# anhtu293/nndepth

Measured on AMD Instinct MI355X. Metric: stereo pairs/sec at 544x960, 32 iters (RAFT-Stereo), higher is better.
Workload: dtype f32 carried as 2 range-scaled fp16 pieces per operand (3 MFMA products, fp32 accumulate); 1 GPU; RAFT-Stereo base (ctx 64), 544x960, 32 iters, batch 1 per GPU, all 32 up_disp emitted; parallelism=single, launch=direct

## Files before the change

### nndepth_amd/csrc/common.h

```cpp
#pragma once
#include <hip/hip_runtime.h>
#include <atomic>
#include <cstdarg>
#include <cstdio>
#include "../../include/nndepth_amd.h"
#include "split_arith.h"

namespace nnd {

void set_error(const char* fmt, ...);

#define NND_HIP_CHECK(expr)                                                              \
    do {                                                                                 \
        hipError_t _e = (expr);                                                          \
        if (_e != hipSuccess) {                                                          \
            nnd::set_error("%s failed: %s (%s:%d)", #expr, hipGetErrorString(_e), __FILE__, __LINE__); \
            return NND_ERR_HIP;                                                          \
        }                                                                                \
    } while (0)

#define NND_LAUNCH_CHECK()                                                               \
    do {                                                                                 \
        hipError_t _e = hipGetLastError();                                               \
        if (_e != hipSuccess) {                                                          \
// ... 97 lines not shown
struct ConvLayer {
    int KH, KW, Cin, Cout, CI_T;
    int stride = 1;
    int arith = 0;
    bool range_scaled() const { return split_range_scaled(arith); }
    int64_t s_off = -1;
    int nchunks;
    int ncb;
    int64_t w_off, b_off;
    int64_t w_floats() const {
        return arith ? (int64_t)ncb * nchunks * KH * KW * arith * 256
                     : (int64_t)ncb * nchunks * KH * KW * CI_T * 32;
    }
    int64_t b_floats() const { return (int64_t)ncb * 32 + (range_scaled() ? 4 : 0); }
    double flops(int B, int H, int W) const { return 2.0 * B * H * W * (double)Cout * Cin * KH * KW; }
    int64_t tail_off() const { return b_off + (int64_t)ncb * 32; }
};

struct Act {
    float* ptr;
    int64_t bstride;
    int C;
};

struct ConvIO {
    Act src0, src1;
    Act out0, out1;
    Act aux0, aux1;
    Act bmap;
    int hidden = 0;
    float scale = 1.f;
    int Hin = 0, Win = 0;
    int flags = 0;
    bool src_tiled = false;
    bool dst_tiled = false;
    bool src_c4 = false;
    bool dst_c4 = false;
    int cout_need = 0;
    int force_ks = 0;
};

static inline bool conv_shape_built(int KH, int KW) { return (KH == 1 && (KW == 1 || KW == 5)) || (KW == 1 && KH == 5) || (KH == 3 && KW == 3); }

int conv_ci_t(int KH, int KW, int Cin, int stride = 1, int Cout = 0);

int launch_conv(const ConvLayer& L, const float* blob, const ConvIO& io, int epi,
                int B, int H, int W, hipStream_t stream);

void pack_conv(const ConvLayer& L, int nparts, const float* const* w, const float* const* b,
               const int* cout, float* blob, const int* ci_map = nullptr, int cin_src = 0);

bool conv_split_supported(int KH, int KW, int Cin, int stride, int arith, int Cout = 0);
int launch_conv_split(const ConvLayer& L, const float* blob, const ConvIO& io, int epi, int B, int H, int W, hipStream_t stream);
bool flow_branch_supported(const ConvLayer& f2, int fc);
int launch_flow_branch(const ConvLayer& f2, const float* blob, const float* w7t, const float* b7, const float* flow, int64_t fbs,
                       int fc, const ConvIO& io, int B, int H, int W, hipStream_t stream);
void pack_conv_split(const ConvLayer& L, int nparts, const float* const* w, const float* const* b, const int* cout, float* blob,
                     const int* ci_map, int cin_src);

bool enc_block_supported(const ConvLayer& c1, const ConvLayer& c2, const ConvLayer& ds);
int enc_block_launch(const ConvLayer& c1, const float* blob1, const ConvLayer& c2, const float* blob2, const ConvLayer& ds, const float* blobd,
                     const float* x, float* out, int N, int H, int W, hipStream_t stream);

bool thin3d_supported(int Cout, int stride);
bool slab3d_supported(int Cout, int C0, int C1, int stride, int arith);
int64_t slab3d_packed_floats(int Cout, int Ct, int stride);
void slab3d_pack(int Cout, int Ct, int stride, const float* w, const float* scale, const float* shift, float* out);
int slab3d_forward(int Cout, int C0, int C1, int stride, const float* packed, const float* x0, const float* x1, float* y, int N, int D,
                   int H, int W, float slope, hipStream_t s);
int64_t thin3d_packed_floats(int Cout, int Ct);
void thin3d_pack(int Cout, int Ct, const float* w, const float* scale, const float* shift, float* out);
int thin3d_forward(int Cout, int C0, int C1, int stride, const float* packed, const float* x0, const float* x1, float* y, int N, int D,
                   int H, int W, float slope, hipStream_t s);

int corr1d_lookup_launch(const float* pyr, const float* coords, float* out, int B, int H, int W, int num_levels,
                         int radius, hipStream_t stream, bool tiled);
int group_lookup_flat_launch(const float* pyr, const float* coords, float* out, int B, int G, int H, int W, int num_levels, int radius,
                             hipStream_t stream, bool tiled);
int igev_lookup_launch(const float* feat_pyramid, const float* geo_pyramid, const float* coords, float* out, int B, int G, int H,
                       int W, int num_levels, int radius, hipStream_t stream, bool tiled);
int convex_upsample_launch(const float* flow, const float* mask, float* out, int B, int C, int H, int W, int rate,
                           hipStream_t stream, bool tiled);

int agcl_iter_launch(const float* f1, const float* f2, const float* flow, float* warped, float* out, int N, int C, int H,
                     int W, int small_patch, hipStream_t s, bool tiled);
int agcl_offset_launch(const float* f1, const float* f2, const float* flow, const float* extra, float* out, int N, int C, int H,
                       int W, int small_patch, hipStream_t s, bool tiled);
int agcl_check(const char* what, int N, int C, int H, int W);
bool agcl_offset_cl_supported(int C);
int agcl_offset_cl_launch(const float* f1c, const float* f2c, const float* flow, const float* extra, float* out, int N, int C,
                          int H, int W, int small_patch, hipStream_t s, bool tiled);
int nchw_to_nhwc_launch(const float* in, float* out, int N, int C, int P, hipStream_t s);
int lookup_convc1_launch(const float* pyr, const float* geo, int G, const float* coords, const ConvLayer& L, const float* blob,
                         float* c1, int64_t c1_bs, int B, int H, int W, int num_levels, int radius, hipStream_t stream, bool c1_c4);
bool flow_branch_lookup_supported(int arith);
int flow_branch_lookup_launch(const ConvLayer& f2, const float* blob, const float* w7t, const float* b7, const float* flow, int64_t fbs,
                              int fc, const ConvIO& io, const float* pyr, const float* coords, const ConvLayer& Lc1, float* c1,
                              int64_t c1_bs, int B, int H, int W, int num_levels, int radius, hipStream_t stream, bool c1_c4);
bool igev_lookup_convc1_il_supported(int G, int num_levels, int radius);
int igev_lookup_convc1_il_launch(const float* il, int G, const float* coords, const ConvLayer& L, const float* blob, float* c1,
                                 int64_t c1_bs, int B, int H, int W, int num_levels, int radius, hipStream_t stream, bool c1_c4);
struct MaskUpFlowHead {
    const float* x;
    long xbs;
    int hid;
    const float* w;
    const float* bias;
    const float* coords_in;
    float *coords_out, *flow_out, *delta_out;
    float* hx_flow;
    long hx_bs;
    int hx_pm;
    int absolute;
};

// ... 8 lines not shown
```

### nndepth_amd/csrc/conv_split.hip

```cpp
#include "conv_launch.h"
#include "conv_split_kernel.h"
#include "flow_branch.h"

#include <atomic>
#include <cmath>
#include <cstdlib>
#include <cstring>

namespace nnd {

namespace {
uint16_t f16_rn(float x) {
    const _Float16 h = (_Float16)x;
    uint16_t u;
    memcpy(&u, &h, 2);
    return u;
}
float f16_to_f(uint16_t u) {
    _Float16 h;
    memcpy(&h, &u, 2);
    return (float)h;
}
uint16_t bf16_rn(float x) {
    uint32_t u;
// ... 57 lines not shown
                    size_t lds = (size_t)2 * ks * P * subb;
                    const size_t red = ks > 1 ? (size_t)waves * P * 4096 : 0;
                    if (red > lds) lds = red;
                    if (lds > 160 * 1024) continue;
                    const int max_waves = P > 2 ? 8 : SPLIT_MAX_WAVES;
                    int wg_per_cu = (int)((160 * 1024) / lds);
                    if (wg_per_cu > max_waves / waves) wg_per_cu = max_waves / waves;
                    if (wg_per_cu < 1) wg_per_cu = 1;
                    const double rounds = std::ceil((double)px_wgs * ny / (256.0 * wg_per_cu));
                    const double simd_waves = std::ceil(waves * wg_per_cu / 4.0);
                    double t = rounds * simd_waves * cdiv(L.nchunks, ks) * P / 2.0;
                    t *= 1.0 + 0.03 * (ks - 1);
                    t *= 1.0 + 0.02 * (4 - (wco < 4 ? wco : 4));
                    if (nu > 2 && P == 2) t *= 1.2;
                    if (t < best) {
                        best = t;
                        *out = {ny, wco, ks, P, ntiles, tiles_x, split_nu_variant(nu), fast, lds, STR};
                        found = true;
                    }
                }
            }
        }
        return found;
    };
    if (try_ks2 && search(force_ny, 2, force_p)) return true;
    if (search(force_ny, force_ks, force_p)) return true;
    return rule && search(-1, -1, -1);
}

bool restrict_split(const ConvLayer& L, int cout_need, SplitCfg* cfg) {
    const int npos = split_patch(L.KH, L.KW, L.arith, L.stride).NPOS;
    auto units = [&](int wco) { return split_staging_units(cfg->P, npos, cfg->ks, wco * cfg->ks); };
    if (!conv_restrict_cout(L, cout_need, &cfg->ny, &cfg->wco, [&](int wco) { return cfg->P == 2 && units(wco) <= 4; })) return false;
    cfg->nu = split_nu_variant(units(cfg->wco));
    return true;
}

bool split_fast_ok(const ConvLayer& L) { return !switches().split_no_fast || L.stride == 2; }
bool plan_split(const ConvLayer& L, const ConvIO& io, int B, int H, int W, SplitCfg* cfg) {
    if (!pick_split(L, io.src0.C, io.src1.C, B, H, W, split_fast_ok(L), cfg)) return false;
    cfg->restricted = restrict_split(L, io.cout_need, cfg);
    cfg->grid = dim3(cdiv(cfg->ntiles, cfg->P), cfg->ny, B), cfg->block = dim3(64 * cfg->wco * cfg->ks);
    return true;
}

void print_split_plan(const ConvLayer& L, const ConvIO& io, const SplitCfg& cfg) {
    fprintf(stderr, "[nnd] conv_split %dx%d Cin=%d Cout=%d pieces=%d: ny=%d, wco=%d, ks=%d, P=%d, nu=%d%s, grid %ux%ux%u, lds %zu B%s%s\n", L.KH,
            L.KW, L.Cin, L.Cout, L.arith, cfg.ny, cfg.wco, cfg.ks, cfg.P, cfg.nu, cfg.fast ? ", fast" : "", cfg.grid.x, cfg.grid.y, cfg.grid.z, cfg.lds,
            io.cout_need > 0 ? (cfg.restricted ? ", restricted to the wanted output channels" : ", whole layer (not restrictable)") : "",
            L.stride == 2 ? ", stride 2" : "");
}
}

extern template int launch_split_ns<1>(const ConvArgs&, const SplitCfg&, int, int, hipStream_t);
extern template int launch_split_ns<2>(const ConvArgs&, const SplitCfg&, int, int, hipStream_t);
extern template int launch_split_ns<3>(const ConvArgs&, const SplitCfg&, int, int, hipStream_t);

bool conv_split_supported(int KH, int KW, int Cin, int stride, int arith, int Cout) {
    if ((arith != 3 && arith != 2 && arith != 1) || (stride != 1 && stride != 2) || Cin % 16 != 0) return false;
    if (stride == 2) return ((KH == 3 && KW == 3) || (KH == 1 && KW == 1)) && Cout >= 96;
    return conv_shape_built(KH, KW);
}

int launch_conv_split(const ConvLayer& L, const float* blob, const ConvIO& io, int epi, int B, int H, int W, hipStream_t stream) {
    int rc, Hin, Win;
    NND_REQUIRE(conv_split_supported(L.KH, L.KW, L.Cin, L.stride, L.arith, L.Cout), "conv_split: %dx%d Cin=%d Cout=%d stride %d arith %d not built",
                L.KH, L.KW, L.Cin, L.Cout, L.stride, L.arith);
    NND_TRY(conv_check_io("conv_split", L, io, epi, H, W, &Hin, &Win));
    NND_REQUIRE(L.CI_T == 16 && L.nchunks * 16 == L.Cin, "conv_split: layer was not planned for 16-channel chunks");
    NND_REQUIRE(L.stride == 1 || io.src1.C == 0, "conv_split: stride 2 is built for one source");
    NND_REQUIRE((long)(L.Cin + 64) * tiled_plane(Hin, Win) < (1L << 31), "conv_split: plane offsets exceed 32 bits");
    SplitCfg cfg;
    NND_REQUIRE(plan_split(L, io, B, H, W, &cfg),
                "conv_split: no configuration for %dx%d Cin=%d (%d+%d) Cout=%d stride %d (NND_SPLIT_CFG ny=%d ks=%d P=%d%s)", L.KH, L.KW,
                L.Cin, io.src0.C, io.src1.C, L.Cout, L.stride, switches().split_ny, switches().split_ks, switches().split_p,
                split_fast_ok(L) ? "" : ", NND_SPLIT_NO_FAST");
    ConvArgs a;
    conv_fill_args(L, blob, io, epi, H, W, Hin, Win, &a);
    a.tiles_x = cfg.tiles_x; a.wco = cfg.wco; a.ks = cfg.ks; a.npos = cfg.ntiles;
#ifdef NND_DBG_STAMPS
    {
        static std::atomic<int> launches{0};
        static const int only = getenv("NND_DBG_STAMP_LAUNCH") ? atoi(getenv("NND_DBG_STAMP_LAUNCH")) : -1;
        const int idx = launches.fetch_add(1);
        a.dbg_stamp = only < 0 || idx == only;
    }
#endif
    if (calibrating() && split_range_scaled(L.arith))
        for (const Act* src : {&io.src0, &io.src1}) NND_TRY(calib_amax_act(*src, a.ls, B, Hin, Win, blob + L.tail_off(), stream));
    if (switches().conv_verbose) print_split_plan(L, io, cfg);
    rc = L.arith == 3   ? launch_split_ns<3>(a, cfg, L.KH, L.KW, stream)
         : L.arith == 2 ? launch_split_ns<2>(a, cfg, L.KH, L.KW, stream)
                        : launch_split_ns<1>(a, cfg, L.KH, L.KW, stream);
    NND_REQUIRE(rc != NND_ERR_UNSUPPORTED, "conv_split: shape %dx%d P=%d nu=%d %s is not instantiated", L.KH, L.KW, cfg.P, cfg.nu, cfg.fast ? "fast" : "generic");
    if (rc != NND_OK) return rc;
    NND_LAUNCH_CHECK();
    return NND_OK;
}

void pack_conv_split(const ConvLayer& L, int nparts, const float* const* w, const float* const* bvec, const int* cout, float* blob,
                     const int* ci_map, int cin_src) {
    if (!ci_map) cin_src = L.Cin;
    const int NT = L.KH * L.KW, NS = L.arith;
    uint16_t* wp = reinterpret_cast<uint16_t*>(blob + L.w_off);
    float* bp = blob + L.b_off;
    memset(wp, 0, sizeof(float) * L.w_floats());
// ... 97 lines not shown
```

### nndepth_amd/csrc/enc_block.hip

```cpp
#include "common.h"
#include "conv_epilogue.h"
#include "conv_split_kernel.h"
#include "layout.h"
#include "split_arith.h"

#include <atomic>

namespace nnd {

namespace {
constexpr int EB_TH = 8, EB_TW = 16;
constexpr int EB_YR = EB_TH + 2, EB_YC = EB_TW + 2;
constexpr int EB_XR = EB_TH + 4, EB_XC = EB_TW + 4;
constexpr int EB_NY = EB_YR * EB_YC, EB_NX = EB_XR * EB_XC;
constexpr int EB_NCH = 4;
constexpr int EB_B1 = 6, EB_B2 = 4;
constexpr int EB_HV = 2;
static_assert(EB_B1 * 32 >= EB_NY && EB_B2 * 32 == EB_TH * EB_TW, "column blocks cover the y region / the tile");
constexpr int eb_ps(int NS) { return NS * 32 + 16; }
constexpr size_t eb_lds_bytes(int NS) { return (size_t)(EB_NCH * EB_NY + EB_NX) * eb_ps(NS); }

struct EncBlockArgs {
    const float* x;
    float* out;
    long bs;
    const uint4 *w1, *w2;
    const float4* wd;
    const float *shift1, *scale1, *shift2, *scale2, *shiftd, *scaled;
    Lay lay;
    int H, W, tiles_x;
};

template <int NS, int P, int RW, int PAR>
__device__ __forceinline__ void eb_walk_chunk(const uint4* wc, const uint4* wn, uint4 (&ab)[2][3][NS], const unsigned char* const (&bb)[P],
                                              f32x16 (&acc)[P]) {
    constexpr int PS = eb_ps(NS), NUNIT = 9 * P;
    uint4 b[2][NS];
    auto read_b = [&](int u, uint4(&dst)[NS]) {
        const int t = u / P, pp = u % P;
#pragma unroll
        for (int s = 0; s < NS; ++s) dst[s] = *reinterpret_cast<const uint4*>(bb[pp] + ((t / 3) * RW + t % 3) * PS + s * 32);
    };
    read_b(0, b[0]);
#pragma unroll
    for (int dy = 0; dy < 3; ++dy) {
        uint4(&cur)[3][NS] = ab[(PAR + dy) & 1];
        uint4(&nxt)[3][NS] = ab[(PAR + dy + 1) & 1];
        const uint4* wr = dy < 2 ? wc + (dy + 1) * 3 * NS * 64 : wn;
#pragma unroll
        for (int dx = 0; dx < 3; ++dx)
#pragma unroll
            for (int s = 0; s < NS; ++s) nxt[dx][s] = wr[(dx * NS + s) * 64];
        __builtin_amdgcn_sched_barrier(0);
#pragma unroll
        for (int dx = 0; dx < 3; ++dx)
#pragma unroll
            for (int pp = 0; pp < P; ++pp) {
                const int u = (dy * 3 + dx) * P + pp;
                if (u + 1 < NUNIT) read_b(u + 1, b[(u + 1) & 1]);
                __builtin_amdgcn_sched_barrier(0);
                split_mfma_step<NS>(cur[dx], b[u & 1], acc[pp]);
                __builtin_amdgcn_sched_barrier(0);
            }
    }
}

template <int NS>
__global__ void __launch_bounds__(128 * EB_HV) __attribute__((amdgpu_waves_per_eu(EB_HV))) enc_block_kernel(EncBlockArgs a) {
    constexpr int EB_P1 = EB_B1 / EB_HV, EB_P2 = EB_B2 / EB_HV, NTHR = 128 * EB_HV, NU = (2 * EB_NX + NTHR - 1) / NTHR;
    constexpr int PS = eb_ps(NS), YCH = EB_NY * PS, CHW = 9 * NS * 64;
    extern __shared__ __attribute__((aligned(16))) unsigned char lds_raw[];
    unsigned char* const ybuf = lds_raw;
    unsigned char* const xbuf = lds_raw + EB_NCH * YCH;

    const int tid = threadIdx.x, lane = tid & 63;
    const int wave = __builtin_amdgcn_readfirstlane(tid >> 6);
    const int cb = wave & 1, half = wave >> 1;
    const int h2 = lane >> 5, l31 = lane & 31;
    const int b = blockIdx.z;
    const int ty0 = (blockIdx.x / a.tiles_x) * EB_TH, tx0 = (blockIdx.x % a.tiles_x) * EB_TW;
    const int H = a.H, W = a.W;
    const int SP = (int)a.lay.plane;
    const float* xs = a.x + b * a.bs;

    int goff[NU], gstep[NU], loff[NU];
    bool inimg[NU], own[NU];
#pragma unroll
    for (int i = 0; i < NU; ++i) {
        const int u = tid + i * NTHR;
        own[i] = u < 2 * EB_NX;
        const int oct = u / EB_NX, pos = u % EB_NX;
        const int gy = ty0 - 2 + pos / EB_XC, gx = tx0 - 2 + pos % EB_XC;
        inimg[i] = own[i] && gy >= 0 && gy < H && gx >= 0 && gx < W;
        goff[i] = inimg[i] ? oct * 8 * SP + (int)pix_off(a.lay, gy, gx) : 0;
        gstep[i] = inimg[i] ? 4 * SP : 0;
        loff[i] = pos * PS + oct * 16;
    }
    float stage[NU][8];
    auto stage_load = [&](int K) {
        const float* src = xs + (long)K * 16 * SP;
#pragma unroll
        for (int i = 0; i < NU; ++i)
#pragma unroll
            for (int g = 0; g < 2; ++g) {
                const float4 t = *reinterpret_cast<const float4*>(src + (unsigned)(goff[i] + g * gstep[i]));
                stage[i][4 * g] = t.x; stage[i][4 * g + 1] = t.y; stage[i][4 * g + 2] = t.z; stage[i][4 * g + 3] = t.w;
            }
    };
    const float* tail1 = a.shift1 + 64;
    const float* tail2 = a.shift2 + 64;
    const float oscale1 = tail1[SPLIT_TAIL_OSCALE], xscale1 = tail1[SPLIT_TAIL_XSCALE];
    const float oscale2 = tail2[SPLIT_TAIL_OSCALE], xscale2 = tail2[SPLIT_TAIL_XSCALE];
    auto stage_store = [&]() {
#pragma unroll
        for (int i = 0; i < NU; ++i) {
            float v[8];
#pragma unroll
            for (int j = 0; j < 8; ++j) v[j] = inimg[i] ? stage[i][j] : 0.f;
            uint4 pieces[NS];
            split_pieces<NS>(v, pieces, xscale1);
            if (own[i]) {
#pragma unroll
                for (int s = 0; s < NS; ++s) *reinterpret_cast<uint4*>(xbuf + loff[i] + s * 32) = pieces[s];
            }
        }
    };

    const unsigned char* xb1[EB_P1];
    int ypos[EB_P1];
    bool ywrite[EB_P1], yin[EB_P1];
#pragma unroll
    for (int pp = 0; pp < EB_P1; ++pp) {
        const int p = (half * EB_P1 + pp) * 32 + l31;
        const int pc = min(p, EB_NY - 1);
        const int yr = pc / EB_YC, yc = pc % EB_YC;
        ypos[pp] = pc;
        ywrite[pp] = p < EB_NY;
        const int iy = ty0 - 1 + yr, ix = tx0 - 1 + yc;
        yin[pp] = iy >= 0 && iy < H && ix >= 0 && ix < W;
        xb1[pp] = xbuf + (yr * EB_XC + yc) * PS + h2 * 16;
    }
    const uint4* w1 = a.w1 + (size_t)cb * EB_NCH * CHW + lane;
    const uint4* w2 = a.w2 + (size_t)cb * EB_NCH * CHW + lane;

    uint4 ab[2][3][NS];
#pragma unroll
    for (int dx = 0; dx < 3; ++dx)
#pragma unroll
        for (int s = 0; s < NS; ++s) ab[0][dx][s] = w1[(dx * NS + s) * 64];
    stage_load(0);
    stage_store();
    __syncthreads();

    f32x16 acc1[EB_P1];
#pragma unroll
    for (int pp = 0; pp < EB_P1; ++pp)
#pragma unroll
        for (int i = 0; i < 16; ++i) acc1[pp][i] = 0.f;

    auto conv1_chunk = [&](int K, auto par_c) {
        constexpr int PAR = decltype(par_c)::value;
        const bool more = K + 1 < EB_NCH;
        if (more) stage_load(K + 1);
        eb_walk_chunk<NS, EB_P1, EB_XC, PAR>(w1 + K * CHW, more ? w1 + (K + 1) * CHW : w2, ab, xb1, acc1);
        __syncthreads();
        if (more) {
            stage_store();
            __syncthreads();
        }
    };
    for (int K = 0; K < EB_NCH; K += 2) {
        conv1_chunk(K, std::integral_constant<int, 0>{});
        conv1_chunk(K + 1, std::integral_constant<int, 1>{});
    }

    {
        float sc1[16], sh1[16];
#pragma unroll
        for (int reg = 0; reg < 16; ++reg) {
            const int co = cb * 32 + (reg & 3) + 8 * (reg >> 2) + 4 * h2;
            sc1[reg] = a.scale1[co];
            sh1[reg] = a.shift1[co];
        }
#pragma unroll
        for (int pp = 0; pp < EB_P1; ++pp) {
#pragma unroll
            for (int q = 0; q < 4; ++q) {
                float v[4];
#pragma unroll
                for (int i = 0; i < 4; ++i) {
                    const float ac = acc1[pp][4 * q + i] * oscale1;
                    const float t = relu_nan(fmaf(ac, sc1[4 * q + i], sh1[4 * q + i]));
                    v[i] = yin[pp] ? t : 0.f;
                }
                uint2 pieces[NS];
                split_pieces_n<NS, 4, uint2>(v, pieces, xscale2);
                if (ywrite[pp]) {
                    unsigned char* d = ybuf + (cb * 2 + (q >> 1)) * YCH + ypos[pp] * PS + ((q & 1) * 8 + 4 * h2) * 2;
#pragma unroll
                    for (int s = 0; s < NS; ++s) *reinterpret_cast<uint2*>(d + s * 32) = pieces[s];
                }
            }
        }
    }
    __syncthreads();

    const int pxl = lane_pixel(l31), r2 = pxl >> 4, c2 = pxl & 15;
    int oy[EB_P2];
    const int ox = tx0 + c2;
    int yb2[EB_P2];
#pragma unroll
    for (int pp = 0; pp < EB_P2; ++pp) {
        const int row = 2 * (half * EB_P2 + pp) + r2;
        oy[pp] = ty0 + row;
        yb2[pp] = (row * EB_YC + c2) * PS + h2 * 16;
    }
    f32x16 acc2[EB_P2];
#pragma unroll
    for (int pp = 0; pp < EB_P2; ++pp)
#pragma unroll
        for (int i = 0; i < 16; ++i) acc2[pp][i] = 0.f;
    float4 xq[EB_P2][8], afr[8];
    auto conv2_chunk = [&](int K, auto par_c) {
        constexpr int PAR = decltype(par_c)::value;
        const unsigned char* bb[EB_P2];
#pragma unroll
        for (int pp = 0; pp < EB_P2; ++pp) bb[pp] = ybuf + K * YCH + yb2[pp];
        eb_walk_chunk<NS, EB_P2, EB_YC, PAR>(w2 + K * CHW, w2 + (K + 1 < EB_NCH ? K + 1 : K) * CHW, ab, bb, acc2);
    };
    conv2_chunk(0, std::integral_constant<int, 0>{});
    conv2_chunk(1, std::integral_constant<int, 1>{});
    conv2_chunk(2, std::integral_constant<int, 0>{});
    {
        const float4* wq = a.wd + (size_t)cb * 8 * 64 + lane;
#pragma unroll
        for (int q = 0; q < 8; ++q) afr[q] = wq[q * 64];
#pragma unroll
        for (int pp = 0; pp < EB_P2; ++pp) {
            const bool ok = oy[pp] < H && ox < W;
            const float* src = xs + (ok ? pix_off(a.lay, oy[pp], ox) : 0);
#pragma unroll
            for (int j = 0; j < 8; ++j) xq[pp][j] = *reinterpret_cast<const float4*>(src + (long)(2 * j + h2) * 4 * SP);
        }
    }
    conv2_chunk(3, std::integral_constant<int, 1>{});

    float scd[16], shd[16], sc2[16], sh2[16];
#pragma unroll
    for (int reg = 0; reg < 16; ++reg) {
        const int co = cb * 32 + (reg & 3) + 8 * (reg >> 2) + 4 * h2;
        scd[reg] = a.scaled[co];
        shd[reg] = a.shiftd[co];
        sc2[reg] = a.scale2[co];
        sh2[reg] = a.shift2[co];
    }
#pragma unroll
    for (int pp = 0; pp < EB_P2; ++pp) {
        float bv[32];
#pragma unroll
        for (int j = 0; j < 8; ++j) {
            const float4 q4 = xq[pp][j];
            const auto s01 = __builtin_amdgcn_permlane32_swap(__float_as_uint(q4.x), __float_as_uint(q4.y), false, false);
            const auto s23 = __builtin_amdgcn_permlane32_swap(__float_as_uint(q4.z), __float_as_uint(q4.w), false, false);
            bv[4 * j + 0] = __uint_as_float(s01[0]);
            bv[4 * j + 1] = __uint_as_float(s23[0]);
            bv[4 * j + 2] = __uint_as_float(s01[1]);
            bv[4 * j + 3] = __uint_as_float(s23[1]);
        }
        f32x16 accs;
#pragma unroll
        for (int i = 0; i < 16; ++i) accs[i] = 0.f;
#pragma unroll
        for (int kp = 0; kp < 32; ++kp) {
            const float4 av = afr[kp / 4];
            const float a_s = (kp % 4 == 0) ? av.x : (kp % 4 == 1) ? av.y : (kp % 4 == 2) ? av.z : av.w;
            accs = __builtin_amdgcn_mfma_f32_32x32x2f32(a_s, bv[kp], accs, 0, 0, 0);
        }
        const bool ok = oy[pp] < H && ox < W;
        float* o = a.out + b * a.bs + (ok ? pix_off(a.lay, oy[pp], ox) : 0);
#pragma unroll
        for (int q = 0; q < 4; ++q) {
            const int co0 = cb * 32 + 8 * q + 4 * h2;
            float v[4];
#pragma unroll
            for (int i = 0; i < 4; ++i) {
                const int reg = 4 * q + i;
                const float ac = acc2[pp][reg] * oscale2;
                float y2 = relu_nan(fmaf(ac, sc2[reg], sh2[reg]));
                const float sc = fmaf(accs[reg], scd[reg], shd[reg]);
                y2 = sc + y2;
                v[i] = relu_nan(y2);
            }
            if (ok) *reinterpret_cast<float4*>(o + (long)co0 * SP) = make_float4(v[0], v[1], v[2], v[3]);
        }
    }
}

template <int NS>
int launch_enc_block(const EncBlockArgs& a, dim3 grid, hipStream_t stream) {
    auto kern = enc_block_kernel<NS>;
    constexpr size_t lds = eb_lds_bytes(NS);
    if (lds > 64 * 1024) {
        static std::atomic<unsigned> raised{0};
        if (int rc = raise_lds_limit(reinterpret_cast<const void*>(kern), raised, (int)lds)) return rc;
    }
    hipLaunchKernelGGL(kern, grid, dim3(128 * EB_HV), lds, stream, a);
    return NND_OK;
}
}

bool enc_block_supported(const ConvLayer& c1, const ConvLayer& c2, const ConvLayer& ds) {
    auto k33 = [](const ConvLayer& l) { return l.KH == 3 && l.KW == 3 && l.Cin == 64 && l.Cout == 64 && l.stride == 1 && l.CI_T == 16 && l.s_off >= 0; };
    return k33(c1) && k33(c2) && c1.arith == c2.arith && (c1.arith == 2 || c1.arith == 1) && ds.KH == 1 && ds.KW == 1 && ds.Cin == 64 &&
           ds.Cout == 64 && ds.stride == 1 && ds.arith == 0 && ds.CI_T == 32 && ds.s_off >= 0;
}

int enc_block_launch(const ConvLayer& c1, const float* blob1, const ConvLayer& c2, const float* blob2, const ConvLayer& ds, const float* blobd,
                     const float* x, float* out, int N, int H, int W, hipStream_t stream) {
    NND_REQUIRE(enc_block_supported(c1, c2, ds), "enc_block: built for 3x3 64 -> 64 convs in fp16x2 / fp16 with an exact 1x1 shortcut");
    NND_REQUIRE(x && out && x != out && N > 0 && H > 0 && W > 0, "enc_block: bad argument");
    NND_REQUIRE(64 * tiled_plane(H, W) < (1L << 31), "enc_block: plane offsets exceed 32 bits");
    EncBlockArgs a{};
    a.x = x; a.out = out;
    a.lay = make_lay(H, W, true, true);
    a.bs = 64 * a.lay.plane;
    a.w1 = reinterpret_cast<const uint4*>(blob1 + c1.w_off); a.shift1 = blob1 + c1.b_off; a.scale1 = blob1 + c1.s_off;
    a.w2 = reinterpret_cast<const uint4*>(blob2 + c2.w_off); a.shift2 = blob2 + c2.b_off; a.scale2 = blob2 + c2.s_off;
    a.wd = reinterpret_cast<const float4*>(blobd + ds.w_off); a.shiftd = blobd + ds.b_off; a.scaled = blobd + ds.s_off;
    a.H = H; a.W = W; a.tiles_x = cdiv(W, EB_TW);
    const dim3 grid(a.tiles_x * cdiv(H, EB_TH), 1, N);
    if (switches().conv_verbose) fprintf(stderr, "[nnd] enc_block 64 -> 64 pieces=%d: grid %ux1x%d, lds %zu B\n", c1.arith, grid.x, N, eb_lds_bytes(c1.arith));
    int rc = c1.arith == 2 ? launch_enc_block<2>(a, grid, stream) : launch_enc_block<1>(a, grid, stream);
    if (rc != NND_OK) return rc;
    NND_LAUNCH_CHECK();
    return NND_OK;
}

}
```

### nndepth_amd/csrc/encoder.hip

```cpp
#include "common.h"
#include "conv_layer.h"
#include "layout.h"

#include <cstdint>
#include <cstring>
#include <vector>

namespace nnd {

static int conv_layer(const nnd_conv_desc* d, ConvLayer* L, int64_t* total, int arith = 0) {
    NND_REQUIRE(d, "conv: null descriptor");
    NND_REQUIRE(d->Cout > 0 && d->Cin > 0, "conv: bad channel counts");
    NND_REQUIRE(d->stride == 1 || d->stride == 2, "conv: stride %d not supported (1, 2)", d->stride);
    const bool k11 = d->KH == 1 && d->KW == 1, k33 = d->KH == 3 && d->KW == 3;
    if (d->stride == 2)
        NND_REQUIRE(k11 || k33, "conv: stride 2 is built for 1x1 and 3x3 kernels");
    else
        NND_REQUIRE(k11 || k33 || (d->KH == 1 && d->KW == 5) || (d->KH == 5 && d->KW == 1),
                    "conv: kernel %dx%d not built (1x1, 3x3, 1x5, 5x1)", d->KH, d->KW);
    if (k11 && d->stride == 1) arith = 0;
    int64_t off = 0;
    *L = make_conv_layer(d->KH, d->KW, d->Cin, d->Cout, d->stride, arith, 0, true, &off);
    if (total) *total = off;
    return NND_OK;
// ... 577 lines not shown
                                         "conv2", "cnet_proj"};
    static_assert(sizeof(kNames) / sizeof(kNames[0]) == 1 + 3 * ENC_BLOCKS + 2, "one name per unit");
    EncPlan p;
    if (make_enc_plan(desc, &p) != NND_OK) return "";
    return (which >= 0 && which < p.units) ? kNames[which] : "";
}

int nnd_encoder_forward(const nnd_encoder_desc* desc, const float* packed, const float* frames, float* fmap, float* cnet_out,
                        int n_cnet, float* workspace, int N, int H, int W, void* stream) {
    return nnd_encoder_forward2(desc, packed, frames, nullptr, N, fmap, cnet_out, n_cnet, workspace, N, H, W, stream);
}

int nnd_encoder_forward2(const nnd_encoder_desc* desc, const float* packed, const float* frames, const float* frames_b, int nsplit,
                         float* fmap, float* cnet_out, int n_cnet, float* workspace, int N, int H, int W, void* stream) {
    EncPlan p;
    int rc = make_enc_plan(desc, &p);
    if (rc != NND_OK) return rc;
    NND_REQUIRE(packed && frames && fmap && workspace && N > 0 && H > 0 && W > 0, "encoder_forward: bad argument");
    NND_REQUIRE(!frames_b || (nsplit > 0 && nsplit < N), "encoder_forward2: a second frame tensor needs 0 < nsplit < N");
    NND_REQUIRE(!cnet_out || (desc->cnet_dim > 0 && n_cnet > 0 && n_cnet <= N), "encoder_forward: cnet_out needs cnet_dim > 0 and 0 < n_cnet <= N");
    CalibScope calib((desc->flags & NND_FLAG_CALIBRATE) && split_range_scaled(desc->arithmetic));
    hipStream_t s = (hipStream_t)stream;
    const int64_t bufsz = enc_buf_floats(N, H, W);
    float* buf[4] = {workspace, workspace + bufsz, workspace + 2 * bufsz, workspace + 3 * bufsz};
    int h = (H + 1) / 2, w = (W + 1) / 2;
    const bool inorm = desc->norm == 2;
    const float eps = 1e-5f;
    float* st_a = workspace + 4 * bufsz;
    float* st_b = st_a + (int64_t)N * 256;
    float* st_c = st_b + (int64_t)N * 256;
    double* part = reinterpret_cast<double*>(st_c + (int64_t)N * 256);
    const bool c4 = desc->arithmetic != 0 && !switches().enc_no_c4;
    {
        const Lay lay = make_lay(h, w, true, c4);
        const int tiles_x = cdiv(w, 32), tiles_y = cdiv(h, 8);
        hipLaunchKernelGGL(stem_kernel, dim3(tiles_x * tiles_y, 1, N), dim3(256), 0, s, frames, frames_b, frames_b ? nsplit : N, packed + p.stem_w,
                           packed + p.stem_scale, packed + p.stem_shift, buf[0], (long)(64 * lay.plane), H, W, h, w, tiles_x, lay,
                           inorm ? 0 : 1);
        NND_LAUNCH_CHECK();
    }
    int cur = 0;
    if (inorm) {
        NND_TRY(in_stats(buf[0], 64 * tiled_plane(h, w), N, 64, h, w, eps, st_a, part, s, c4));
        NND_TRY(in_apply(buf[0], 64 * tiled_plane(h, w), st_a, nullptr, 0, nullptr, N, 64, h, w, true, s, c4));
    }
    for (int i = 0; i < ENC_BLOCKS; ++i) {
        const int st = p.strides[i], cin = p.inpl[i], dim = p.planes[i];
        const int ho = (h + st - 1) / st, wo = (w + st - 1) / st;
        const int64_t pin = tiled_plane(h, w), pout = tiled_plane(ho, wo);
        float* x = buf[cur];
        float* y = buf[(cur + 1) & 3];
        float* sc = buf[(cur + 2) & 3];
        float* o = buf[(cur + 3) & 3];
        const bool fused = !inorm && c4 && st == 1 && !calibrating() && !switches().no_fused_enc_block && enc_block_supported(p.c1[i], p.c2[i], p.ds[i]);
        if (fused) {
            NND_TRY(enc_block_launch(p.c1[i], packed + p.base1[i], p.c2[i], packed + p.base2[i], p.ds[i], packed + p.based[i], x, o, N, h, w, s));
        } else if (!inorm) {
            NND_TRY(run_conv_norm(p.c1[i], packed + p.base1[i], x, cin * pin, true, nullptr, 0, y, dim * pout, true, 1, N, h, w, s, c4, c4));
            NND_TRY(run_conv_norm(p.ds[i], packed + p.based[i], x, cin * pin, true, nullptr, 0, sc, dim * pout, true, 0, N, h, w, s, c4, c4));
            NND_TRY(run_conv_norm(p.c2[i], packed + p.base2[i], y, dim * pout, true, sc, dim * pout, o, dim * pout, true, 3, N, ho, wo, s, c4, c4));
        } else {
            NND_TRY(run_conv_norm(p.c1[i], packed + p.base1[i], x, cin * pin, true, nullptr, 0, y, dim * pout, true, 0, N, h, w, s, c4, c4));
            NND_TRY(in_stats(y, dim * pout, N, dim, ho, wo, eps, st_a, part, s, c4));
            NND_TRY(in_apply(y, dim * pout, st_a, nullptr, 0, nullptr, N, dim, ho, wo, true, s, c4));
            NND_TRY(run_conv_norm(p.ds[i], packed + p.based[i], x, cin * pin, true, nullptr, 0, sc, dim * pout, true, 0, N, h, w, s, c4, c4));
            NND_TRY(in_stats(sc, dim * pout, N, dim, ho, wo, eps, st_b, part, s, c4));
            NND_TRY(run_conv_norm(p.c2[i], packed + p.base2[i], y, dim * pout, true, nullptr, 0, o, dim * pout, true, 0, N, ho, wo, s, c4, c4));
            NND_TRY(in_stats(o, dim * pout, N, dim, ho, wo, eps, st_c, part, s, c4));
            NND_TRY(in_apply(o, dim * pout, st_c, sc, dim * pout, st_b, N, dim, ho, wo, true, s, c4));
        }
        cur = (cur + 3) & 3;
        h = ho; w = wo;
    }
    const int64_t pl = tiled_plane(h, w);
    NND_TRY(run_conv_norm(p.out, packed + p.base_out, buf[cur], 128 * pl, true, nullptr, 0, fmap, (int64_t)desc->output_dim * h * w,
                          false, 0, N, h, w, s, c4, false));
    if (cnet_out)
        NND_TRY(run_conv_norm(p.cnet, packed + p.base_cnet, fmap, (int64_t)desc->output_dim * h * w, false, nullptr, 0, cnet_out,
                              (int64_t)desc->cnet_dim * h * w, false, 1, n_cnet, h, w, s));
    return NND_OK;
}

}
```

Measured before the change: 142.5 pairs/s.

## Extend fused encoder residual block kernel to 96-channel and stride-2 blocks

Generalizes the fused encoder residual-block kernel (conv1 + conv2 + 1x1 shortcut in one launch) through a templated shape struct. It now also covers the 96->96 stride-1 blocks and the 64->96 stride-2 downsampling block, which uses a phase-split input layout in LDS and a split-precision MFMA shortcut. The aim is to cut launches and the global round trips of intermediate activations in the encoder's second stage. The fused path is used only when none of the convs would pick split-K, because the fused kernel gives up that extra parallelism.

```diff
diff --git a/nndepth_amd/csrc/common.h b/nndepth_amd/csrc/common.h
--- a/nndepth_amd/csrc/common.h
+++ b/nndepth_amd/csrc/common.h
@@ -173,6 +173,7 @@
 
 bool conv_split_supported(int KH, int KW, int Cin, int stride, int arith, int Cout = 0);
 int launch_conv_split(const ConvLayer& L, const float* blob, const ConvIO& io, int epi, int B, int H, int W, hipStream_t stream);
+bool conv_split_no_split_k(const ConvLayer& L, int B, int H, int W);
 bool flow_branch_supported(const ConvLayer& f2, int fc);
 int launch_flow_branch(const ConvLayer& f2, const float* blob, const float* w7t, const float* b7, const float* flow, int64_t fbs,
                        int fc, const ConvIO& io, int B, int H, int W, hipStream_t stream);
@@ -181,7 +182,7 @@
 
 bool enc_block_supported(const ConvLayer& c1, const ConvLayer& c2, const ConvLayer& ds);
 int enc_block_launch(const ConvLayer& c1, const float* blob1, const ConvLayer& c2, const float* blob2, const ConvLayer& ds, const float* blobd,
-                     const float* x, float* out, int N, int H, int W, hipStream_t stream);
+                     const float* x, float* out, int N, int Hx, int Wx, hipStream_t stream);
 
 bool thin3d_supported(int Cout, int stride);
 bool slab3d_supported(int Cout, int C0, int C1, int stride, int arith);
diff --git a/nndepth_amd/csrc/conv_split.hip b/nndepth_amd/csrc/conv_split.hip
--- a/nndepth_amd/csrc/conv_split.hip
+++ b/nndepth_amd/csrc/conv_split.hip
@@ -133,6 +133,11 @@
 }
 }
 
+bool conv_split_no_split_k(const ConvLayer& L, int B, int H, int W) {
+    SplitCfg cfg;
+    return pick_split(L, L.Cin, 0, B, H, W, split_fast_ok(L), &cfg) && cfg.ks == 1;
+}
+
 extern template int launch_split_ns<1>(const ConvArgs&, const SplitCfg&, int, int, hipStream_t);
 extern template int launch_split_ns<2>(const ConvArgs&, const SplitCfg&, int, int, hipStream_t);
 extern template int launch_split_ns<3>(const ConvArgs&, const SplitCfg&, int, int, hipStream_t);
diff --git a/nndepth_amd/csrc/enc_block.hip b/nndepth_amd/csrc/enc_block.hip
--- a/nndepth_amd/csrc/enc_block.hip
+++ b/nndepth_amd/csrc/enc_block.hip
@@ -9,37 +9,46 @@
 namespace nnd {
 
 namespace {
-constexpr int EB_TH = 8, EB_TW = 16;
-constexpr int EB_YR = EB_TH + 2, EB_YC = EB_TW + 2;
-constexpr int EB_XR = EB_TH + 4, EB_XC = EB_TW + 4;
-constexpr int EB_NY = EB_YR * EB_YC, EB_NX = EB_XR * EB_XC;
-constexpr int EB_NCH = 4;
-constexpr int EB_B1 = 6, EB_B2 = 4;
-constexpr int EB_HV = 2;
-static_assert(EB_B1 * 32 >= EB_NY && EB_B2 * 32 == EB_TH * EB_TW, "column blocks cover the y region / the tile");
+template <int NCB_, int CIN_, int STR_>
+struct EbShape {
+    static constexpr int NCB = NCB_, C = 32 * NCB, NCH = 2 * NCB, CIN = CIN_, NCH1 = CIN / 16, STR = STR_;
+    static constexpr int NQ = CIN / 8;
+    static constexpr int TH = 8, TW = 16;
+    static constexpr int YR = TH + 2, YC = TW + 2, NY = YR * YC;
+    static constexpr int XR = TH + 4, XC = TW + 4;
+    static constexpr int XRW = STR == 1 ? XC : YC + 1, PHN = STR == 1 ? 0 : (YR + 1) * XRW, NX = STR == 1 ? XR * XC : 4 * PHN;
+    static constexpr int B1 = 6, B2 = 4;
+    static constexpr int HV = 2;
+    static constexpr int P1 = B1 / HV, P2 = B2 / HV, NTHR = 64 * NCB * HV;
+    static_assert(B1 * 32 >= NY && B2 * 32 == TH * TW, "column blocks cover the y region / the tile");
+    static_assert((STR == 1 && CIN == C) || STR == 2, "a stride-1 block keeps its channel count");
+    static_assert(NCH1 % 2 == 0, "the weight ring's phase returns to 0 behind conv1");
+    static constexpr size_t lds_bytes(int NS) { return (size_t)(NCH * NY + NX) * (NS * 32 + 16); }
+};
 constexpr int eb_ps(int NS) { return NS * 32 + 16; }
-constexpr size_t eb_lds_bytes(int NS) { return (size_t)(EB_NCH * EB_NY + EB_NX) * eb_ps(NS); }
 
 struct EncBlockArgs {
     const float* x;
     float* out;
-    long bs;
+    long bsx, bs;
     const uint4 *w1, *w2;
     const float4* wd;
     const float *shift1, *scale1, *shift2, *scale2, *shiftd, *scaled;
-    Lay lay;
-    int H, W, tiles_x;
+    Lay layx, lay;
+    int Hx, Wx, H, W, tiles_x;
 };
 
-template <int NS, int P, int RW, int PAR>
+template <int NS, int P, int RW, int PAR, int PHN = 0>
 __device__ __forceinline__ void eb_walk_chunk(const uint4* wc, const uint4* wn, uint4 (&ab)[2][3][NS], const unsigned char* const (&bb)[P],
                                               f32x16 (&acc)[P]) {
     constexpr int PS = eb_ps(NS), NUNIT = 9 * P;
     uint4 b[2][NS];
     auto read_b = [&](int u, uint4(&dst)[NS]) {
         const int t = u / P, pp = u % P;
-#pragma unroll
-        for (int s = 0; s < NS; ++s) dst[s] = *reinterpret_cast<const uint4*>(bb[pp] + ((t / 3) * RW + t % 3) * PS + s * 32);
+        const int dy = t / 3, dx = t % 3;
+        const int toff = PHN == 0 ? dy * RW + dx : ((dy & 1) * 2 + (dx & 1)) * PHN + (dy >> 1) * RW + (dx >> 1);
+#pragma unroll
+        for (int s = 0; s < NS; ++s) dst[s] = *reinterpret_cast<const uint4*>(bb[pp] + toff * PS + s * 32);
     };
     read_b(0, b[0]);
 #pragma unroll
@@ -65,9 +74,11 @@
     }
 }
 
-template <int NS>
-__global__ void __launch_bounds__(128 * EB_HV) __attribute__((amdgpu_waves_per_eu(EB_HV))) enc_block_kernel(EncBlockArgs a) {
-    constexpr int EB_P1 = EB_B1 / EB_HV, EB_P2 = EB_B2 / EB_HV, NTHR = 128 * EB_HV, NU = (2 * EB_NX + NTHR - 1) / NTHR;
+template <int NS, class S>
+__global__ void __launch_bounds__(S::NTHR) __attribute__((amdgpu_waves_per_eu(2))) enc_block_kernel(EncBlockArgs a) {
+    constexpr int EB_P1 = S::P1, EB_P2 = S::P2, NTHR = S::NTHR, NU = (2 * S::NX + NTHR - 1) / NTHR;
+    constexpr int EB_TH = S::TH, EB_TW = S::TW, EB_YC = S::YC, EB_XC = S::XC, EB_NY = S::NY, EB_NX = S::NX, EB_NCH = S::NCH;
+    constexpr int NCB = S::NCB, C = S::C, NQ = S::NQ, STR = S::STR, NCH1 = S::NCH1, XRW = S::XRW, PHN = S::PHN;
     constexpr int PS = eb_ps(NS), YCH = EB_NY * PS, CHW = 9 * NS * 64;
     extern __shared__ __attribute__((aligned(16))) unsigned char lds_raw[];
     unsigned char* const ybuf = lds_raw;
@@ -75,13 +86,13 @@
 
     const int tid = threadIdx.x, lane = tid & 63;
     const int wave = __builtin_amdgcn_readfirstlane(tid >> 6);
-    const int cb = wave & 1, half = wave >> 1;
+    const int cb = wave % NCB, half = wave / NCB;
     const int h2 = lane >> 5, l31 = lane & 31;
     const int b = blockIdx.z;
     const int ty0 = (blockIdx.x / a.tiles_x) * EB_TH, tx0 = (blockIdx.x % a.tiles_x) * EB_TW;
     const int H = a.H, W = a.W;
-    const int SP = (int)a.lay.plane;
-    const float* xs = a.x + b * a.bs;
+    const int SP = (int)a.lay.plane, SPX = (int)a.layx.plane;
+    const float* xs = a.x + b * a.bsx;
 
     int goff[NU], gstep[NU], loff[NU];
     bool inimg[NU], own[NU];
@@ -90,15 +101,21 @@
         const int u = tid + i * NTHR;
         own[i] = u < 2 * EB_NX;
         const int oct = u / EB_NX, pos = u % EB_NX;
-        const int gy = ty0 - 2 + pos / EB_XC, gx = tx0 - 2 + pos % EB_XC;
-        inimg[i] = own[i] && gy >= 0 && gy < H && gx >= 0 && gx < W;
-        goff[i] = inimg[i] ? oct * 8 * SP + (int)pix_off(a.lay, gy, gx) : 0;
-        gstep[i] = inimg[i] ? 4 * SP : 0;
+        int gy, gx;
+        if constexpr (STR == 1) {
+            gy = ty0 - 2 + pos / EB_XC, gx = tx0 - 2 + pos % EB_XC;
+        } else {
+            const int ph = pos / PHN, q = pos % PHN;
+            gy = 2 * ty0 - 3 + 2 * (q / XRW) + (ph >> 1), gx = 2 * tx0 - 3 + 2 * (q % XRW) + (ph & 1);
+        }
+        inimg[i] = own[i] && gy >= 0 && gy < a.Hx && gx >= 0 && gx < a.Wx;
+        goff[i] = inimg[i] ? oct * 8 * SPX + (int)pix_off(a.layx, gy, gx) : 0;
+        gstep[i] = inimg[i] ? 4 * SPX : 0;
         loff[i] = pos * PS + oct * 16;
     }
     float stage[NU][8];
     auto stage_load = [&](int K) {
-        const float* src = xs + (long)K * 16 * SP;
+        const float* src = xs + (long)K * 16 * SPX;
 #pragma unroll
         for (int i = 0; i < NU; ++i)
 #pragma unroll
@@ -107,8 +124,8 @@
                 stage[i][4 * g] = t.x; stage[i][4 * g + 1] = t.y; stage[i][4 * g + 2] = t.z; stage[i][4 * g + 3] = t.w;
             }
     };
-    const float* tail1 = a.shift1 + 64;
-    const float* tail2 = a.shift2 + 64;
+    const float* tail1 = a.shift1 + C;
+    const float* tail2 = a.shift2 + C;
     const float oscale1 = tail1[SPLIT_TAIL_OSCALE], xscale1 = tail1[SPLIT_TAIL_XSCALE];
     const float oscale2 = tail2[SPLIT_TAIL_OSCALE], xscale2 = tail2[SPLIT_TAIL_XSCALE];
     auto stage_store = [&]() {
@@ -138,9 +155,9 @@
         ywrite[pp] = p < EB_NY;
         const int iy = ty0 - 1 + yr, ix = tx0 - 1 + yc;
         yin[pp] = iy >= 0 && iy < H && ix >= 0 && ix < W;
-        xb1[pp] = xbuf + (yr * EB_XC + yc) * PS + h2 * 16;
-    }
-    const uint4* w1 = a.w1 + (size_t)cb * EB_NCH * CHW + lane;
+        xb1[pp] = xbuf + (yr * XRW + yc) * PS + h2 * 16;
+    }
+    const uint4* w1 = a.w1 + (size_t)cb * NCH1 * CHW + lane;
     const uint4* w2 = a.w2 + (size_t)cb * EB_NCH * CHW + lane;
 
     uint4 ab[2][3][NS];
@@ -160,16 +177,16 @@
 
     auto conv1_chunk = [&](int K, auto par_c) {
         constexpr int PAR = decltype(par_c)::value;
-        const bool more = K + 1 < EB_NCH;
+        const bool more = K + 1 < NCH1;
         if (more) stage_load(K + 1);
-        eb_walk_chunk<NS, EB_P1, EB_XC, PAR>(w1 + K * CHW, more ? w1 + (K + 1) * CHW : w2, ab, xb1, acc1);
+        eb_walk_chunk<NS, EB_P1, XRW, PAR, PHN>(w1 + K * CHW, more ? w1 + (K + 1) * CHW : w2, ab, xb1, acc1);
         __syncthreads();
         if (more) {
             stage_store();
             __syncthreads();
         }
     };
-    for (int K = 0; K < EB_NCH; K += 2) {
+    for (int K = 0; K < NCH1; K += 2) {
         conv1_chunk(K, std::integral_constant<int, 0>{});
         conv1_chunk(K + 1, std::integral_constant<int, 1>{});
     }
@@ -220,7 +237,8 @@
     for (int pp = 0; pp < EB_P2; ++pp)
 #pragma unroll
         for (int i = 0; i < 16; ++i) acc2[pp][i] = 0.f;
-    float4 xq[EB_P2][8], afr[8];
+    constexpr int NXQ = STR == 1 ? NQ : 2 * NCH1, NAF = STR == 1 ? NQ : NCH1 * NS;
+    float4 xq[EB_P2][NXQ], afr[NAF];
     auto conv2_chunk = [&](int K, auto par_c) {
         constexpr int PAR = decltype(par_c)::value;
         const unsigned char* bb[EB_P2];
@@ -228,23 +246,33 @@
         for (int pp = 0; pp < EB_P2; ++pp) bb[pp] = ybuf + K * YCH + yb2[pp];
         eb_walk_chunk<NS, EB_P2, EB_YC, PAR>(w2 + K * CHW, w2 + (K + 1 < EB_NCH ? K + 1 : K) * CHW, ab, bb, acc2);
     };
-    conv2_chunk(0, std::integral_constant<int, 0>{});
-    conv2_chunk(1, std::integral_constant<int, 1>{});
-    conv2_chunk(2, std::integral_constant<int, 0>{});
+    for (int K = 0; K < EB_NCH - 2; K += 2) {
+        conv2_chunk(K, std::integral_constant<int, 0>{});
+        conv2_chunk(K + 1, std::integral_constant<int, 1>{});
+    }
+    conv2_chunk(EB_NCH - 2, std::integral_constant<int, 0>{});
+    constexpr int NAE = NAF < 8 ? NAF : 8;
+    const float4* wq = a.wd + (size_t)cb * NAF * 64 + lane;
     {
-        const float4* wq = a.wd + (size_t)cb * 8 * 64 + lane;
-#pragma unroll
-        for (int q = 0; q < 8; ++q) afr[q] = wq[q * 64];
+#pragma unroll
+        for (int q = 0; q < NAE; ++q) afr[q] = wq[q * 64];
 #pragma unroll
         for (int pp = 0; pp < EB_P2; ++pp) {
             const bool ok = oy[pp] < H && ox < W;
-            const float* src = xs + (ok ? pix_off(a.lay, oy[pp], ox) : 0);
-#pragma unroll
-            for (int j = 0; j < 8; ++j) xq[pp][j] = *reinterpret_cast<const float4*>(src + (long)(2 * j + h2) * 4 * SP);
-        }
-    }
-    conv2_chunk(3, std::integral_constant<int, 1>{});
-
+            const float* src = xs + (ok ? pix_off(a.layx, STR * oy[pp], STR * ox) : 0);
+#pragma unroll
+            for (int j = 0; j < NXQ; ++j) {
+                const int quad = STR == 1 ? 2 * j + h2 : 4 * (j / 2) + 2 * h2 + j % 2;
+                xq[pp][j] = *reinterpret_cast<const float4*>(src + (long)quad * 4 * SPX);
+            }
+        }
+    }
+    conv2_chunk(EB_NCH - 1, std::integral_constant<int, 1>{});
+#pragma unroll
+    for (int q = NAE; q < NAF; ++q) afr[q] = wq[q * 64];
+
+    const float* taild = a.shiftd + C;
+    const float oscaled = STR == 1 ? 1.f : taild[SPLIT_TAIL_OSCALE], xscaled = STR == 1 ? 1.f : taild[SPLIT_TAIL_XSCALE];
     float scd[16], shd[16], sc2[16], sh2[16];
 #pragma unroll
     for (int reg = 0; reg < 16; ++reg) {
@@ -256,9 +284,24 @@
     }
 #pragma unroll
     for (int pp = 0; pp < EB_P2; ++pp) {
-        float bv[32];
-#pragma unroll
-        for (int j = 0; j < 8; ++j) {
+        f32x16 accs;
+#pragma unroll
+        for (int i = 0; i < 16; ++i) accs[i] = 0.f;
+        if constexpr (STR == 2) {
+#pragma unroll
+            for (int K = 0; K < NCH1; ++K) {
+                const float4 lo = xq[pp][2 * K], hi = xq[pp][2 * K + 1];
+                const float v[8] = {lo.x, lo.y, lo.z, lo.w, hi.x, hi.y, hi.z, hi.w};
+                uint4 pieces[NS], aw[NS];
+                split_pieces<NS>(v, pieces, xscaled);
+#pragma unroll
+                for (int s = 0; s < NS; ++s) aw[s] = __builtin_bit_cast(uint4, afr[K * NS + s]);
+                split_mfma_step<NS>(aw, pieces, accs);
+            }
+        } else {
+        float bv[4 * NQ];
+#pragma unroll
+        for (int j = 0; j < NQ; ++j) {
             const float4 q4 = xq[pp][j];
             const auto s01 = __builtin_amdgcn_permlane32_swap(__float_as_uint(q4.x), __float_as_uint(q4.y), false, false);
             const auto s23 = __builtin_amdgcn_permlane32_swap(__float_as_uint(q4.z), __float_as_uint(q4.w), false, false);
@@ -267,14 +310,12 @@
             bv[4 * j + 2] = __uint_as_float(s01[1]);
             bv[4 * j + 3] = __uint_as_float(s23[1]);
         }
-        f32x16 accs;
-#pragma unroll
-        for (int i = 0; i < 16; ++i) accs[i] = 0.f;
-#pragma unroll
-        for (int kp = 0; kp < 32; ++kp) {
+#pragma unroll
+        for (int kp = 0; kp < 4 * NQ; ++kp) {
             const float4 av = afr[kp / 4];
             const float a_s = (kp % 4 == 0) ? av.x : (kp % 4 == 1) ? av.y : (kp % 4 == 2) ? av.z : av.w;
             accs = __builtin_amdgcn_mfma_f32_32x32x2f32(a_s, bv[kp], accs, 0, 0, 0);
+        }
         }
         const bool ok = oy[pp] < H && ox < W;
         float* o = a.out + b * a.bs + (ok ? pix_off(a.lay, oy[pp], ox) : 0);
@@ -287,7 +328,7 @@
                 const int reg = 4 * q + i;
                 const float ac = acc2[pp][reg] * oscale2;
                 float y2 = relu_nan(fmaf(ac, sc2[reg], sh2[reg]));
-                const float sc = fmaf(accs[reg], scd[reg], shd[reg]);
+                const float sc = fmaf(STR == 1 ? accs[reg] : accs[reg] * oscaled, scd[reg], shd[reg]);
                 y2 = sc + y2;
                 v[i] = relu_nan(y2);
             }
@@ -296,44 +337,61 @@
     }
 }
 
-template <int NS>
+template <int NS, class S>
 int launch_enc_block(const EncBlockArgs& a, dim3 grid, hipStream_t stream) {
-    auto kern = enc_block_kernel<NS>;
-    constexpr size_t lds = eb_lds_bytes(NS);
+    auto kern = enc_block_kernel<NS, S>;
+    constexpr size_t lds = S::lds_bytes(NS);
     if (lds > 64 * 1024) {
         static std::atomic<unsigned> raised{0};
         if (int rc = raise_lds_limit(reinterpret_cast<const void*>(kern), raised, (int)lds)) return rc;
     }
-    hipLaunchKernelGGL(kern, grid, dim3(128 * EB_HV), lds, stream, a);
+    hipLaunchKernelGGL(kern, grid, dim3(S::NTHR), lds, stream, a);
     return NND_OK;
 }
-}
-
-bool enc_block_supported(const ConvLayer& c1, const ConvLayer& c2, const ConvLayer& ds) {
-    auto k33 = [](const ConvLayer& l) { return l.KH == 3 && l.KW == 3 && l.Cin == 64 && l.Cout == 64 && l.stride == 1 && l.CI_T == 16 && l.s_off >= 0; };
-    return k33(c1) && k33(c2) && c1.arith == c2.arith && (c1.arith == 2 || c1.arith == 1) && ds.KH == 1 && ds.KW == 1 && ds.Cin == 64 &&
-           ds.Cout == 64 && ds.stride == 1 && ds.arith == 0 && ds.CI_T == 32 && ds.s_off >= 0;
-}
-
-int enc_block_launch(const ConvLayer& c1, const float* blob1, const ConvLayer& c2, const float* blob2, const ConvLayer& ds, const float* blobd,
-                     const float* x, float* out, int N, int H, int W, hipStream_t stream) {
-    NND_REQUIRE(enc_block_supported(c1, c2, ds), "enc_block: built for 3x3 64 -> 64 convs in fp16x2 / fp16 with an exact 1x1 shortcut");
-    NND_REQUIRE(x && out && x != out && N > 0 && H > 0 && W > 0, "enc_block: bad argument");
-    NND_REQUIRE(64 * tiled_plane(H, W) < (1L << 31), "enc_block: plane offsets exceed 32 bits");
+
+template <class S>
+int enc_block_run(const ConvLayer& c1, const float* blob1, const ConvLayer& c2, const float* blob2, const ConvLayer& ds, const float* blobd,
+                  const float* x, float* out, int N, int Hx, int Wx, hipStream_t stream) {
+    const int H = cdiv(Hx, S::STR), W = cdiv(Wx, S::STR);
     EncBlockArgs a{};
     a.x = x; a.out = out;
-    a.lay = make_lay(H, W, true, true);
-    a.bs = 64 * a.lay.plane;
+    a.layx = make_lay(Hx, Wx, true, true); a.lay = make_lay(H, W, true, true);
+    a.bsx = S::CIN * a.layx.plane; a.bs = S::C * a.lay.plane;
     a.w1 = reinterpret_cast<const uint4*>(blob1 + c1.w_off); a.shift1 = blob1 + c1.b_off; a.scale1 = blob1 + c1.s_off;
     a.w2 = reinterpret_cast<const uint4*>(blob2 + c2.w_off); a.shift2 = blob2 + c2.b_off; a.scale2 = blob2 + c2.s_off;
     a.wd = reinterpret_cast<const float4*>(blobd + ds.w_off); a.shiftd = blobd + ds.b_off; a.scaled = blobd + ds.s_off;
-    a.H = H; a.W = W; a.tiles_x = cdiv(W, EB_TW);
-    const dim3 grid(a.tiles_x * cdiv(H, EB_TH), 1, N);
-    if (switches().conv_verbose) fprintf(stderr, "[nnd] enc_block 64 -> 64 pieces=%d: grid %ux1x%d, lds %zu B\n", c1.arith, grid.x, N, eb_lds_bytes(c1.arith));
-    int rc = c1.arith == 2 ? launch_enc_block<2>(a, grid, stream) : launch_enc_block<1>(a, grid, stream);
+    a.Hx = Hx; a.Wx = Wx; a.H = H; a.W = W; a.tiles_x = cdiv(W, S::TW);
+    const dim3 grid(a.tiles_x * cdiv(H, S::TH), 1, N);
+    if (switches().conv_verbose)
+        fprintf(stderr, "[nnd] %s %d -> %d stride %d pieces=%d: grid %ux1x%d, lds %zu B\n", S::C == 64 ? "enc_block" : "enc_stage2_block", S::CIN,
+                S::C, S::STR, c1.arith, grid.x, N, S::lds_bytes(c1.arith));
+    int rc = c1.arith == 2 ? launch_enc_block<2, S>(a, grid, stream) : launch_enc_block<1, S>(a, grid, stream);
     if (rc != NND_OK) return rc;
     NND_LAUNCH_CHECK();
     return NND_OK;
 }
-
-}
+}
+
+bool enc_block_supported(const ConvLayer& c1, const ConvLayer& c2, const ConvLayer& ds) {
+    const int Cin = c1.Cin, C = c1.Cout, st = c1.stride;
+    auto conv = [](const ConvLayer& l, int k, int cin, int cout, int stride) {
+        return l.KH == k && l.KW == k && l.Cin == cin && l.Cout == cout && l.stride == stride && l.s_off >= 0;
+    };
+    if (!conv(c1, 3, Cin, C, st) || !conv(c2, 3, C, C, 1) || !conv(ds, 1, Cin, C, st) || c1.CI_T != 16 || c2.CI_T != 16 || c1.arith != c2.arith ||
+        (c1.arith != 2 && c1.arith != 1))
+        return false;
+    if (st == 1) return Cin == C && (C == 64 || C == 96) && ds.arith == 0 && ds.CI_T == 32;
+    return st == 2 && Cin == 64 && C == 96 && ds.arith == c1.arith && ds.CI_T == 16;
+}
+
+int enc_block_launch(const ConvLayer& c1, const float* blob1, const ConvLayer& c2, const float* blob2, const ConvLayer& ds, const float* blobd,
+                     const float* x, float* out, int N, int Hx, int Wx, hipStream_t stream) {
+    NND_REQUIRE(enc_block_supported(c1, c2, ds), "enc_block: built for the 64 -> 64, 96 -> 96 (stride 1) and 64 -> 96 (stride 2) blocks in fp16x2 / fp16");
+    NND_REQUIRE(x && out && x != out && N > 0 && Hx > 0 && Wx > 0, "enc_block: bad argument");
+    NND_REQUIRE(c1.Cout * tiled_plane(Hx, Wx) < (1L << 31), "enc_block: plane offsets exceed 32 bits");
+    if (c1.stride == 2) return enc_block_run<EbShape<3, 64, 2>>(c1, blob1, c2, blob2, ds, blobd, x, out, N, Hx, Wx, stream);
+    if (c1.Cin == 64) return enc_block_run<EbShape<2, 64, 1>>(c1, blob1, c2, blob2, ds, blobd, x, out, N, Hx, Wx, stream);
+    return enc_block_run<EbShape<3, 96, 1>>(c1, blob1, c2, blob2, ds, blobd, x, out, N, Hx, Wx, stream);
+}
+
+}
diff --git a/nndepth_amd/csrc/encoder.hip b/nndepth_amd/csrc/encoder.hip
--- a/nndepth_amd/csrc/encoder.hip
+++ b/nndepth_amd/csrc/encoder.hip
@@ -653,7 +653,9 @@
         float* y = buf[(cur + 1) & 3];
         float* sc = buf[(cur + 2) & 3];
         float* o = buf[(cur + 3) & 3];
-        const bool fused = !inorm && c4 && st == 1 && !calibrating() && !switches().no_fused_enc_block && enc_block_supported(p.c1[i], p.c2[i], p.ds[i]);
+        const bool fused = !inorm && c4 && !calibrating() && !switches().no_fused_enc_block && enc_block_supported(p.c1[i], p.c2[i], p.ds[i]) &&
+                           conv_split_no_split_k(p.c1[i], N, ho, wo) && conv_split_no_split_k(p.c2[i], N, ho, wo) &&
+                           (p.ds[i].arith == 0 || conv_split_no_split_k(p.ds[i], N, ho, wo));
         if (fused) {
             NND_TRY(enc_block_launch(p.c1[i], packed + p.base1[i], p.c2[i], packed + p.base2[i], p.ds[i], packed + p.based[i], x, o, N, h, w, s));
         } else if (!inorm) {
```

After: 144.0 pairs/s, median of 6. +1.1%, better.
